# 0kam/alproj

Hardware: AMD Instinct MI355X
Metric: Gpoints/s projected (pinhole + Brown-Conrady, single pose) over the 100M-vertex DSM; CMA-ES iterations/s in `cma` (higher is better)
Workload: dtype f32

## Files before the change

### alproj_amd/_build.py

```python
import os
import shutil
import subprocess
import sys

HERE = os.path.dirname(os.path.abspath(__file__))
ROOT = os.path.dirname(HERE)
CSRC = os.path.join(HERE, "csrc")
INCLUDE = os.path.join(ROOT, "include")
BUILD = os.path.join(ROOT, "build")
LIB = os.path.join(HERE, "libalproj_hip.so")
SOURCES = ["alp_core.hip", "alp_points.hip", "alp_raster.hip", "alp_mesh.hip", "alp_rasterize.hip", "alp_sampler.hip",
           "alp_cma.hip", "alp_lm.hip", "host/alp_host.cpp"]
HOST_DIR = os.path.join(CSRC, "host")
HOST_SAN = os.path.join(BUILD, "host_san")
HOST_KINDS = {"plain": [], "asan": ["-fsanitize=address,undefined", "-fno-sanitize-recover=all"], "tsan": ["-fsanitize=thread"]}
EXTRA_FLAGS = {"alp_raster.hip": ["-ffp-contract=off"], "alp_mesh.hip": ["-ffp-contract=off"], "alp_cma.hip": ["-ffp-contract=off"],
               "alp_lm.hip": ["-ffp-contract=off"]}
ARCH = "gfx950"


def hipcc():
    exe = shutil.which("hipcc") or "/opt/rocm/bin/hipcc"
    if not os.path.exists(exe):
        raise RuntimeError("hipcc not found; libalproj_hip.so cannot be built")
    return exe


def _stale(target, deps):
    if not os.path.exists(target):
        return True
    t = os.path.getmtime(target)
    return any(os.path.getmtime(d) > t for d in deps)


# ... 38 lines not shown
        return shutil.which("g++")
    exe = "/opt/rocm/lib/llvm/bin/clang++"
    return exe if os.path.exists(exe) else shutil.which("amdclang++")


def build_host(kind="plain", compiler="clang", force=False):
    cxx = host_compiler(compiler)
    if not cxx:
        raise RuntimeError(f"no {compiler} C++ compiler found")
    os.makedirs(HOST_SAN, exist_ok=True)
    srcs = [os.path.join(HOST_DIR, f) for f in ("alp_host.cpp", "alp_host_selfcheck.cpp")]
    deps = srcs + [os.path.join(HOST_DIR, f) for f in ("alp_host.h", "alp_fold.h", "alp_plan.h", "alp_jacplan.h", "alp_lm.h", "alp_buffer.h")] + [os.path.join(INCLUDE, "alproj_hip.h"), os.path.abspath(__file__)]
    exe = os.path.join(HOST_SAN, f"alp_host_{kind}_{compiler}")
    if force or _stale(exe, deps):
        cmd = [cxx, "-O1", "-g", "-fno-omit-frame-pointer", "-std=c++17", "-ffp-contract=off", "-Wall", "-Wextra", f"-I{INCLUDE}", f"-I{CSRC}"] + \
              HOST_KINDS[kind] + srcs + ["-o", exe, "-lpthread"]
        r = subprocess.run(cmd, capture_output=True, text=True)
        if r.returncode != 0:
            sys.stderr.write(r.stderr)
            raise RuntimeError(f"{cxx} failed on the host-only build ({kind})")
    return exe


def resource_usage():
    out = {}
    for src in SOURCES:
        log = os.path.join(BUILD, os.path.basename(src).replace(".hip", ".o.log").replace(".cpp", ".o.log"))
        if not os.path.exists(log):
            continue
        cur = None
        for line in open(log):
            if "remark:" not in line or "[-Rpass-analysis" not in line:
                continue
            body = line.split("remark:", 1)[1].split("[-Rpass")[0].strip()
            if body.startswith("Function Name:"):
                cur = body.split(":", 1)[1].strip()
                out[cur] = {}
            elif cur and ":" in body:
                k, v = body.split(":", 1)
                out[cur][k.strip()] = v.strip()
    return out


if __name__ == "__main__":
    print(build(force="--force" in sys.argv, verbose=True))
    for k, v in resource_usage().items():
# ... 3 lines not shown
```

### alproj_amd/_lib.py

```python
import ctypes
import os
import threading
import weakref

import numpy as np

_HERE = os.path.dirname(os.path.abspath(__file__))
LIB_PATH = os.environ.get("ALPROJ_HIP_LIB", os.path.join(_HERE, "libalproj_hip.so"))

ALP_F32, ALP_F64, ALP_I32, ALP_I64, ALP_U8, ALP_U16 = 0, 1, 2, 3, 4, 5
LOSS_MEAN_DIST, LOSS_HUBER = 0, 1
NORMAL_LOSSES = {"linear": 0, "soft_l1": 1, "huber": 2, "cauchy": 3}
NORMAL_BATCH_MAX = 1024
WEIGHT_TABLE_MAX_BYTES = 1 << 30
NPARAM = 25
UNIQUE_ID_BYTES = 128

PARAM_KEYS = ("x", "y", "z", "fov", "pan", "tilt", "roll", "a1", "a2",
              "k1", "k2", "k3", "k4", "k5", "k6", "p1", "p2",
              "s1", "s2", "s3", "s4", "w", "h", "cx", "cy")
DIST_KEYS = PARAM_KEYS[7:21]


_POOL_MIN = 8 << 20
# ... 128 lines not shown
    "alp_synchronize": [],
    "alp_event_record": [_c_int],
    "alp_event_elapsed_ms": [_c_int, _c_int, _c_fp],
    "alp_kernel_timing": [_c_int],
    "alp_kernel_time_ms": [_c_fp, ctypes.POINTER(_c_int)],
    "alp_build_flags": [],
    "alp_comm_unique_id": [ctypes.c_char_p],
    "alp_comm_init": [ctypes.c_char_p, _c_int, _c_int],
    "alp_comm_destroy": [],
    "alp_comm_info": [ctypes.POINTER(_c_int), ctypes.POINTER(_c_int)],
    "alp_comm_bcast": [_c_void_p, _c_i64, _c_int],
    "alp_comm_allgather_counts": [_c_i64, ctypes.POINTER(_c_i64)],
    "alp_comm_allgatherv": [_c_void_p, _c_void_p, ctypes.POINTER(_c_i64)],
    "alp_points_create": [_c_void_p, _c_int, _c_i64, _c_dp, _c_int, ctypes.POINTER(_c_void_p)],
    "alp_points_create_columns": [_c_void_p, _c_void_p, _c_void_p, _c_int, _c_i64, _c_dp, _c_int, ctypes.POINTER(_c_void_p)],
    "alp_points_destroy": [_c_void_p],
    "alp_points_count": [_c_void_p, ctypes.POINTER(_c_i64)],
    "alp_points_layout": [_c_void_p, ctypes.POINTER(_c_i64)],
    "alp_points_set_observed": [_c_void_p, _c_void_p, _c_int],
    "alp_points_set_observed_columns": [_c_void_p, _c_void_p, _c_void_p, _c_int],
    "alp_project": [_c_void_p, _c_dp],
    "alp_projected_fetch": [_c_void_p, _c_void_p, _c_void_p, _c_int],
    "alp_projected_fetch_strided": [_c_void_p, _c_i64, _c_i64, _c_i64, _c_dp, _c_dp],
    "alp_residuals": [_c_void_p, _c_dp, _c_dp],
    "alp_residuals_batch": [_c_void_p, _c_dp, _c_i64, _c_dp],
    "alp_jacobian": [_c_void_p, _c_dp, ctypes.POINTER(ctypes.c_int32), _c_int, _c_int, _c_dp],
    "alp_normal_equations": [_c_void_p, _c_dp, ctypes.POINTER(ctypes.c_int32), _c_int, _c_int, _c_double, _c_dp],
    "alp_normal_equations_batch": [_c_void_p, _c_dp, _c_i64, ctypes.POINTER(ctypes.c_int32), _c_int, _c_int, _c_double, _c_dp],
    "alp_eval_population": [_c_void_p, _c_dp, _c_i64, _c_int, _c_double, _c_dp, ctypes.POINTER(_c_i64)],
    "alp_eval_population_enqueue": [_c_void_p, _c_dp, _c_i64, _c_int, _c_double],
    "alp_eval_population_wait": [_c_void_p, _c_dp, ctypes.POINTER(_c_i64)],
    "alp_eval_population_timing": [_c_void_p, _c_fp, _c_fp],
    "alp_eval_population_info": [_c_void_p, ctypes.POINTER(_c_i64)],
    "alp_points_set_mend": [_c_void_p, _c_int],
    "alp_points_set_weights": [_c_void_p, _c_void_p, _c_int],
    "alp_points_weight_sum": [_c_void_p, ctypes.POINTER(ctypes.c_double)],
    "alp_points_set_weight_table": [_c_void_p, _c_void_p, _c_int, _c_int],
    "alp_points_weight_table_sums": [_c_void_p, _c_dp],
    "alp_normal_equations_batch_rows": [_c_void_p, _c_dp, _c_i64, ctypes.POINTER(ctypes.c_int32), ctypes.POINTER(ctypes.c_int32), _c_int,
                                        _c_int, _c_double, _c_dp],
    "alp_residuals_assigned": [_c_void_p, _c_dp, _c_i64, ctypes.POINTER(ctypes.c_int32), _c_dp],
    "alp_eval_population_mended": [_c_void_p, ctypes.POINTER(_c_i64)],
    "alp_loss_uv": [_c_dp, _c_dp, _c_i64, _c_int, _c_double, _c_dp],
    "alp_loss_uv_columns": [_c_dp, _c_dp, _c_dp, _c_dp, _c_i64, _c_int, _c_double, _c_dp],
    "alp_cma_sample": [_c_dp, _c_double, _c_dp, _c_dp, _c_dp, _c_int, _c_i64, _c_int, ctypes.c_uint64, ctypes.c_uint64, _c_dp,
                       ctypes.POINTER(ctypes.c_int32)],
# ... 198 lines not shown
    return idx


def weights_check(w, n, precision=None):
    w = np.asarray(w)
    if w.dtype not in (np.float32, np.float64):
        w = w.astype(np.float64)
    w = np.ascontiguousarray(w)
    if w.shape != (n,):
        raise ValueError(f"weights must have shape ({n},)")
    if not np.isfinite(w).all() or (w < 0).any():
        raise ValueError("weights must be finite and >= 0")
    with np.errstate(over="ignore"):
        stored = w.astype(np.float32) if precision == ALP_F32 else w
    if not np.isfinite(stored).all():
        raise ValueError("a weight does not fit float32")
    world = _c_int()
    check(load().alp_comm_info(None, ctypes.byref(world)))
    if world.value == 1 and n > 0 and not stored.astype(np.float64).sum() > 0:
        raise ValueError("the weights sum to 0: no point is left")
    return w


class Points:

    def __init__(self, xyz, origin, precision="f32", _columns=None):
        l = lib()
        cols = _columns
        if cols is None:
            xyz = np.asarray(xyz)
            if xyz.ndim != 2 or xyz.shape[1] != 3:
                raise ValueError("xyz must have shape (N, 3)")
            if xyz.dtype not in (np.float32, np.float64):
                xyz = xyz.astype(np.float64)
            if not xyz.flags["C_CONTIGUOUS"] and xyz.shape[0] > 1 and all(xyz[:, k].flags["C_CONTIGUOUS"] for k in range(3)):
                cols = [xyz[:, k] for k in range(3)]
        self.precision = PRECISIONS[precision]
        self.origin = np.ascontiguousarray(origin, dtype=np.float64).reshape(3)
        h = _c_void_p()
        if cols is not None:
            cols = _same_float_columns(cols, 3)
            self.n = int(len(cols[0]))
            check(l.alp_points_create_columns(*[c.ctypes.data_as(_c_void_p) for c in cols], dtype_code(cols[0]), self.n,
                                              as_dp(self.origin), self.precision, ctypes.byref(h)))
        else:
            xyz = np.ascontiguousarray(xyz)
# ... 789 lines not shown
```

### alproj_amd/csrc/alp_core.hip

```cpp
#include "alp_internal.h"

#include <rccl/rccl.h>
#include <cmath>
#include <cstdlib>
#include <vector>

namespace alp {

Context &ctx() {
    static Context c;
    return c;
}

int require_init() {
    if (!ctx().ready) return fail(ALP_ENOTINIT, "alp_init has not been called (or failed)");
    return ALP_OK;
}

int scratch_reserve(size_t bytes, void **out) {
    Context &c = ctx();
    if (bytes > c.scratch_cap) {
        if (c.scratch) {
            ALP_HIP(hipStreamSynchronize(c.stream));
            hipFree(c.scratch);
// ... 75 lines not shown
    hipError_t e = hipGetDeviceCount(&n);
    if (e != hipSuccess || n <= 0)
        return fail(ALP_ENODEVICE, "no HIP device available (%s); libalproj_hip has no CPU fallback",
                    e == hipSuccess ? "device count is 0" : hipGetErrorString(e));
    if (device < 0 || device >= n)
        return fail(ALP_ENODEVICE, "device %d out of range (have %d)", device, n);
    ALP_HIP(hipSetDevice(device));
    hipDeviceProp_t prop;
    ALP_HIP(hipGetDeviceProperties(&prop, device));
    c.cu_count = prop.multiProcessorCount;
    ALP_HIP(hipStreamCreateWithFlags(&c.stream, hipStreamNonBlocking));
    for (auto &ev : c.events) ALP_HIP(hipEventCreate(&ev));
    c.device = device;
    c.ready = true;
    return ALP_OK;
}

int alp_shutdown(void) {
    Context &c = ctx();
    if (!c.ready) return ALP_OK;
    alp_comm_destroy();
    hipStreamSynchronize(c.stream);
    points_release_staging();
    if (c.scratch) hipFree(c.scratch);
    c.scratch = nullptr;
    c.scratch_cap = 0;
    for (auto &ev : c.events) {
        if (ev) hipEventDestroy(ev);
        ev = nullptr;
    }
    for (int i = 0; i < KT_MAX; ++i) {
        if (g_kt.a[i]) hipEventDestroy(g_kt.a[i]);
        if (g_kt.b[i]) hipEventDestroy(g_kt.b[i]);
        g_kt.a[i] = g_kt.b[i] = nullptr;
    }
    g_kt = KTimer();
    hipStreamDestroy(c.stream);
    c.stream = nullptr;
    c.ready = false;
    c.device = -1;
    return ALP_OK;
}

int alp_device_info(char *name, int len, int *cu_count, int64_t *hbm_bytes) {
    if (int rc = require_init()) return rc;
    hipDeviceProp_t prop;
// ... 194 lines not shown
```

### alproj_amd/csrc/alp_internal.h

```cpp
#pragma once

#include <hip/hip_runtime.h>

#include "host/alp_host.h"
#include "host/alp_buffer.h"

namespace alp {

#define ALP_HIP(expr)                                                                     \
    do {                                                                                  \
        hipError_t e__ = (expr);                                                          \
        if (e__ != hipSuccess)                                                            \
            return ::alp::fail(ALP_EHIP, "%s failed: %s (%s:%d)", #expr,                  \
                               hipGetErrorString(e__), __FILE__, __LINE__);               \
    } while (0)

struct DeviceMemory {
    static int alloc(void **p, size_t bytes) {
        const hipError_t e = hipMalloc(p, bytes);
        return e == hipSuccess ? ALP_OK : fail(ALP_EHIP, "hipMalloc of %zu bytes failed: %s", bytes, hipGetErrorString(e));
    }
    static void release(void *p) { hipFree(p); }
};
struct PinnedMemory {
// ... 31 lines not shown
    hipStream_t stream = nullptr;
    hipEvent_t events[64] = {};
    void *scratch = nullptr;
    size_t scratch_cap = 0;
    void *comm = nullptr;
    int rank = 0;
    int world = 1;
};
Context &ctx();
int require_init();
int scratch_reserve(size_t bytes, void **out);

void ktime_begin();
void ktime_end();
struct KTimeScope {
    KTimeScope() { ktime_begin(); }
    ~KTimeScope() { ktime_end(); }
};


const char *raster_dev_flags();

void points_release_staging();

int comm_allreduce_sum_f64(double *dev_buf, int64_t count);

}
```

### alproj_amd/csrc/alp_point_kernels.h

```cpp
#pragma once

#include "alp_internal.h"

namespace alp {

template <typename T> struct Num;
template <> struct Num<float> {
    using vec = float4;
    static constexpr int VEC = 4;
    static __device__ __forceinline__ float rcp(float a) { return __builtin_amdgcn_rcpf(a); }
    static __device__ __forceinline__ float sqrt(float a) { return __builtin_amdgcn_sqrtf(a); }
    static __device__ __forceinline__ float fma(float a, float b, float c) { return __builtin_fmaf(a, b, c); }
    static __device__ __forceinline__ float rcp_pop(float a) { return rcp(a); }
    static __device__ __forceinline__ float sqrt_pop(float a) { return sqrt(a); }
    typedef float native4 __attribute__((ext_vector_type(4)));
    static __device__ __forceinline__ float4 nt_load(const float4 *p) {
        const native4 t = __builtin_nontemporal_load(reinterpret_cast<const native4 *>(p));
        return make_float4(t.x, t.y, t.z, t.w);
    }
    static __device__ __forceinline__ float4 load(const float4 *p) {
        const native4 t = *reinterpret_cast<const native4 *>(p);
        return make_float4(t.x, t.y, t.z, t.w);
    }
    static __device__ __forceinline__ void nt_store(const float4 &a, float4 *p) {
// ... 643 lines not shown
                                                     const TS *__restrict__ uo, const TS *__restrict__ vo, int64_t n,
                                                     int64_t groups_per, double inv_f_scale, const JacPlan *__restrict__ plan,
                                                     double *__restrict__ partials, const TS *__restrict__ wts) {
    normal_body<TS, LOSS, WEIGHTED>(x, y, z, uo, vo, n, groups_per, inv_f_scale, plan, (int64_t)blockIdx.x, partials, (int64_t)blockIdx.x, wts);
}

constexpr int NORMAL_BATCH_POSE_IN_X = 1;
template <typename TS, int LOSS, bool WEIGHTED = false>
__global__ __launch_bounds__(256) void normal_poses_kernel(const TS *__restrict__ x, const TS *__restrict__ y, const TS *__restrict__ z,
                                                           const TS *__restrict__ uo, const TS *__restrict__ vo, int64_t n,
                                                           int64_t groups_per, double inv_f_scale, const JacPlan *__restrict__ plans,
                                                           const int *__restrict__ list, const long long *__restrict__ count,
                                                           int pose_in_x, double *__restrict__ partials, const TS *__restrict__ wts,
                                                           int64_t row_stride, const int *__restrict__ row_of_pose) {
    const int slot = pose_in_x ? blockIdx.x : blockIdx.y, stripe = pose_in_x ? blockIdx.y : blockIdx.x;
    const int stripes = pose_in_x ? gridDim.y : gridDim.x;
    if (count && (long long)slot >= *count) return;
    const int pose = list ? list[slot] : slot;
    if constexpr (WEIGHTED) wts += (int64_t)(row_of_pose ? row_of_pose[pose] : pose) * row_stride;
    normal_body<TS, LOSS, WEIGHTED>(x, y, z, uo, vo, n, groups_per, inv_f_scale, plans + pose, (int64_t)stripe, partials,
                                    (int64_t)pose * stripes + stripe, wts);
}

__global__ __launch_bounds__(256) void reduce_normal_poses_kernel(const double *__restrict__ partials, int stripes, int T, double n_local,
                                                                  const double *__restrict__ row_sums, const int *__restrict__ row_of_pose,
                                                                  const int *__restrict__ running, double *__restrict__ sums) {
    __shared__ double s[8][32];
    const int cl = threadIdx.x & 31;
    const int g = threadIdx.x >> 5;
    const int c = blockIdx.x * 32 + cl;
    const double *rows = partials + (int64_t)blockIdx.y * stripes * T;
    double *out = sums + (int64_t)blockIdx.y * (T + 1);
    const bool live = running ? running[blockIdx.y] != 0 : true;
    double acc = 0.0;
    if (c < T && live)
        for (int b = g; b < stripes; b += 8) acc += rows[(int64_t)b * T + c];
    s[g][cl] = acc;
    __syncthreads();
    if (g == 0 && c < T) {
        double t = s[0][cl];
#pragma unroll
        for (int k = 1; k < 8; ++k) t += s[k][cl];
        out[c] = t;
    }
    if (blockIdx.x == 0 && threadIdx.x == 0) out[T] = row_sums ? row_sums[row_of_pose ? row_of_pose[blockIdx.y] : (int)blockIdx.y] : n_local;
}


constexpr int64_t WT_SUM_CHUNK = 16384;
template <typename TIn>
__global__ __launch_bounds__(256) void weight_table_sums_kernel(const TIn *__restrict__ src, int64_t row_stride, int64_t len, int64_t chunk,
                                                                double *__restrict__ out) {
    __shared__ double s[256];
    const int tid = threadIdx.x;
    const int64_t beg = (int64_t)blockIdx.x * chunk;
    const int64_t end = beg + chunk < len ? beg + chunk : len;
    const TIn *row = src + (int64_t)blockIdx.y * row_stride;
    double acc = 0.0;
    for (int64_t i = beg + tid; i < end; i += 256) acc += (double)row[i];
    s[tid] = acc;
    __syncthreads();
    for (int m = 128; m >= 1; m >>= 1) {
        if (tid < m) s[tid] += s[tid + m];
        __syncthreads();
    }
    if (tid == 0) out[(int64_t)blockIdx.y * gridDim.x + blockIdx.x] = s[0];
}

constexpr int RA_LDS_POSES = 128;
// ... 147 lines not shown
template <typename T, int LOSS, typename Cfg = PopCfg<T>, bool SHARED_POSE = false, typename TS = T, bool LENS_FREE = false, bool WEIGHTED = false>
__global__ __launch_bounds__(256, Cfg::MINW) void popeval_kernel(
    const TS *__restrict__ x, const TS *__restrict__ y, const TS *__restrict__ z, const TS *__restrict__ uo,
    const TS *__restrict__ vo, int64_t n, const PoseRec<T> *__restrict__ cands, int P, T f_scale,
    double *__restrict__ partials, const PoseRec<T> *__restrict__ cands_general, const TS *__restrict__ wts) {
    popeval_body<T, LOSS, Cfg, SHARED_POSE, TS, LENS_FREE, WEIGHTED>(x, y, z, uo, vo, n, cands, P, f_scale, partials, cands_general, wts);
}

struct MendCount {
    long long last;
    long long total;
};

template <int LOSS, bool WEIGHTED = false>
__global__ __launch_bounds__(256, PopCfg<double>::MINW) void popeval_counted_kernel(
    const float *__restrict__ x, const float *__restrict__ y, const float *__restrict__ z, const float *__restrict__ uo,
    const float *__restrict__ vo, int64_t n, const PoseRec<double> *__restrict__ cands, const MendCount *__restrict__ cnt,
    double f_scale, double *__restrict__ partials, const float *__restrict__ wts) {
    const int count = (int)cnt->last;
    if ((int)blockIdx.y * PopCfg<double>::TC >= count) return;
    popeval_body<double, LOSS, PopCfg<double>, false, float, false, WEIGHTED>(x, y, z, uo, vo, n, cands, count, f_scale, partials, cands, wts);
}

__global__ __launch_bounds__(256) void mend_select_kernel(const double *__restrict__ sums, int P, const double *__restrict__ params,
                                                          double o0, double o1, double o2, int *__restrict__ idx,
                                                          PoseRec<double> *__restrict__ recs, MendCount *__restrict__ cnt) {
    __shared__ int s_wave[4];
    __shared__ int s_base;
    const int tid = threadIdx.x, lane = tid & 63, wave = tid >> 6;
    if (tid == 0) s_base = 0;
    __syncthreads();
    for (int c0 = 0; c0 < P; c0 += 256) {
        const int c = c0 + tid;
        const bool bad = c < P && (__builtin_bit_cast(unsigned long long, sums[c < P ? c : 0]) & 0x7ff0000000000000ull) == 0x7ff0000000000000ull;
        const unsigned long long m = __builtin_amdgcn_ballot_w64(bad);
        if (lane == 0) s_wave[wave] = __builtin_popcountll(m);
        __syncthreads();
        int before = s_base;
        for (int w = 0; w < wave; ++w) before += s_wave[w];
        if (bad) idx[before + __builtin_popcountll(m & ((1ull << lane) - 1ull))] = c;
        __syncthreads();
        if (tid == 0) s_base += (s_wave[0] + s_wave[1]) + (s_wave[2] + s_wave[3]);
        __syncthreads();
    }
    const int count = s_base;
    if (tid == 0) {
// ... 36 lines not shown
    if (k < (int)cnt->last) sums[idx[k]] = mended[k];
}

__global__ __launch_bounds__(256) void reduce_partials_kernel(const double *__restrict__ partials,
                                                              int nblk, int P, double n_local,
                                                              double *__restrict__ sums) {
    __shared__ double s[8][32];
    const int cl = threadIdx.x & 31;
    const int g = threadIdx.x >> 5;
    const int c = blockIdx.x * 32 + cl;
    double acc = 0.0;
    if (c < P)
        for (int b = g; b < nblk; b += 8) acc += partials[(int64_t)b * P + c];
    s[g][cl] = acc;
    __syncthreads();
    if (g == 0 && c < P) {
        double t = s[0][cl];
#pragma unroll
        for (int k = 1; k < 8; ++k) t += s[k][cl];
        sums[c] = t;
    }
    if (blockIdx.x == 0 && threadIdx.x == 0) sums[P] = n_local;
}

template <int LOSS, bool OBS_COLUMNS, bool PRJ_COLUMNS>
__global__ __launch_bounds__(256) void loss_uv_kernel(const double *__restrict__ obs_a, const double *__restrict__ obs_b,
                                                      const double *__restrict__ prj_a, const double *__restrict__ prj_b, int64_t n,
                                                      double f_scale, double *__restrict__ partials) {
    __shared__ double s[4];
    double acc = 0.0;
    const int64_t stride = (int64_t)gridDim.x * blockDim.x;
    for (int64_t i = (int64_t)blockIdx.x * blockDim.x + threadIdx.x; i < n; i += stride) {
        double2 o, q;
        if constexpr (OBS_COLUMNS) o = make_double2(obs_a[i], obs_b[i]);
        else o = reinterpret_cast<const double2 *>(obs_a)[i];
        if constexpr (PRJ_COLUMNS) q = make_double2(prj_a[i], prj_b[i]);
        else q = reinterpret_cast<const double2 *>(prj_a)[i];
        const double du = o.x - q.x, dv = o.y - q.y;
        const double r = __builtin_sqrt(du * du + dv * dv);
        if constexpr (LOSS == ALP_LOSS_MEAN_DIST) acc += r;
        else acc += (r <= f_scale) ? 0.5 * (r * r) : f_scale * (r - 0.5 * f_scale);
    }
    acc = wave_sum_to_lane63(acc);
    if ((threadIdx.x & 63) == 63) s[threadIdx.x >> 6] = acc;
    __syncthreads();
    if (threadIdx.x == 0) partials[blockIdx.x] = ((s[0] + s[1]) + s[2]) + s[3];
}

template <typename TIn, typename T, int C>
__global__ __launch_bounds__(256) void aos_to_planes_kernel(const TIn *__restrict__ src, int64_t count,
                                                            int64_t dst_off, double o0, double o1, double o2,
                                                            T *__restrict__ p0, T *__restrict__ p1,
                                                            T *__restrict__ p2) {
    const int64_t stride = (int64_t)gridDim.x * blockDim.x;
    for (int64_t i = (int64_t)blockIdx.x * blockDim.x + threadIdx.x; i < count; i += stride) {
        p0[dst_off + i] = (T)((double)src[i * C + 0] - o0);
        p1[dst_off + i] = (T)((double)src[i * C + 1] - o1);
        if constexpr (C == 3) p2[dst_off + i] = (T)((double)src[i * C + 2] - o2);
    }
}

template <typename T>
__global__ __launch_bounds__(256) void gather_strided_kernel(const T *__restrict__ u, const T *__restrict__ v,
                                                             int64_t first, int64_t stride, int64_t count,
                                                             double *__restrict__ out) {
    const int64_t i = (int64_t)blockIdx.x * blockDim.x + threadIdx.x;
    if (i < count) {
        out[i] = (double)u[first + i * stride];
        out[count + i] = (double)v[first + i * stride];
    }
}

}
```

### alproj_amd/optimize.py

```python
from contextlib import nullcontext
from math import cos, pi, sin, tan

import numpy as np
import pandas as pd
from scipy.optimize import least_squares
from tqdm import tqdm

from . import _lib, resample
from .cma import CMA

__all__ = ["intrinsic_mat", "extrinsic_mat", "project", "rmse", "huber_loss",
           "compute_residuals", "DEFAULT_BOUND_WIDTHS", "bounds_to_array", "BaseOptimizer",
           "CMAOptimizer", "LsqOptimizer", "start_seeds", "best_start", "normal_lm", "normal_lm_batch"]


def intrinsic_mat(fov_x_deg, w, h, cx=None, cy=None):
    if cx is None:
        cx = w / 2
    if cy is None:
        cy = h / 2
    half_x = fov_x_deg * pi / 180 / 2
    half_y = (fov_x_deg * pi / 180) * h / w / 2
    return np.array([[w / (2 * tan(half_x)), 0, cx],
                     [0, h / (2 * tan(half_y)), cy],
# ... 62 lines not shown
    if isinstance(uv, list):
        pts.set_observed_columns(uv[0], uv[1])
    else:
        pts.set_observed(uv)


def _as_rows(a):
    return np.ascontiguousarray(np.column_stack(a) if isinstance(a, list) else a, dtype=np.float64)


F64_MAX_POINTS = 4_000_000


def default_precision(n_points, precision=None):
    if precision is not None:
        if precision not in ("f32", "f64"):
            raise ValueError("precision must be None, 'f32' or 'f64'")
        return precision
    return "f64" if int(n_points) <= F64_MAX_POINTS else "f32"


def project(obj_points, params, precision="f64"):
    xyz = _xyz_array(obj_points)
    with _points(xyz, _camera_origin(params), precision) as pts:
        pts.project(_lib.params_vector(params))
        u, v = pts.fetch(np.float64)
    return pd.DataFrame({"u": u, "v": v}, copy=False)


def _uv_pointers(a):
    if isinstance(a, list):
        cols = [np.ascontiguousarray(c, dtype=np.float64) for c in a]
        return _lib.as_dp(cols[0]), _lib.as_dp(cols[1]), len(cols[0]), cols
    a = np.asarray(a, dtype=np.float64)
    if a.ndim != 2 or a.shape[1] != 2:
        raise ValueError("pixel coordinates must have shape (N, 2)")
    if not a.flags["C_CONTIGUOUS"] and a.shape[0] > 1 and a[:, 0].flags["C_CONTIGUOUS"] and a[:, 1].flags["C_CONTIGUOUS"]:
        cols = [a[:, 0], a[:, 1]]
        return _lib.as_dp(cols[0]), _lib.as_dp(cols[1]), a.shape[0], cols
    a = np.ascontiguousarray(a)
    return _lib.as_dp(a), None, a.shape[0], a


def _loss_uv(img_points, projected, kind, f_scale):
    prj = _first_two_columns(projected) if isinstance(projected, pd.DataFrame) else projected
    ou, ov, n_obs, keep_o = _uv_pointers(_uv_array(img_points))
    pu, pv, n_prj, keep_p = _uv_pointers(prj)
    if n_obs != n_prj:
        raise ValueError("img_points and projected must have the same shape")
# ... 702 lines not shown
```

### include/alproj_hip.h

```cpp
#ifndef ALPROJ_HIP_H
#define ALPROJ_HIP_H

#include <stdint.h>

#ifdef __cplusplus
extern "C" {
#endif

#define ALP_ABI_VERSION 7

#define ALP_NPARAM 25
#define ALP_PARAM_ORDER "x,y,z,fov,pan,tilt,roll,a1,a2,k1,k2,k3,k4,k5,k6,p1,p2,s1,s2,s3,s4,w,h,cx,cy"

enum alp_error {
    ALP_OK = 0,
    ALP_EINVAL = -1,
    ALP_ENOTINIT = -2,
    ALP_ENODEVICE = -3,
    ALP_EHIP = -4,
    ALP_ERCCL = -5,
    ALP_ESTATE = -6
};

enum alp_dtype {
// ... 44 lines not shown
int alp_comm_init(const char id[ALP_UNIQUE_ID_BYTES], int rank, int world_size);
int alp_comm_destroy(void);
int alp_comm_info(int *rank, int *world_size);
int alp_comm_bcast(void *buf, int64_t bytes, int root);
int alp_comm_allgather_counts(int64_t bytes, int64_t *counts);
int alp_comm_allgatherv(const void *send, void *recv, const int64_t *counts);

typedef struct alp_points alp_points_t;

int alp_points_create(const void *xyz, int in_dtype, int64_t n, const double origin[3],
                      int precision, alp_points_t **out);
int alp_points_create_columns(const void *x, const void *y, const void *z, int in_dtype, int64_t n,
                              const double origin[3], int precision, alp_points_t **out);
int alp_points_destroy(alp_points_t *pts);
int alp_points_count(const alp_points_t *pts, int64_t *n);
int alp_points_layout(const alp_points_t *pts, int64_t *row_length);
int alp_points_set_observed(alp_points_t *pts, const void *uv, int in_dtype);
int alp_points_set_observed_columns(alp_points_t *pts, const void *u, const void *v, int in_dtype);

int alp_project(alp_points_t *pts, const double params[ALP_NPARAM]);
int alp_projected_fetch(alp_points_t *pts, void *u_out, void *v_out, int out_dtype);
int alp_projected_fetch_strided(alp_points_t *pts, int64_t first, int64_t stride,
                                int64_t count, double *u_out, double *v_out);

int alp_residuals(alp_points_t *pts, const double params[ALP_NPARAM], double *out);
int alp_residuals_batch(alp_points_t *pts, const double *cand, int64_t B, double *out);
int alp_jacobian(alp_points_t *pts, const double params[ALP_NPARAM], const int32_t *target_idx, int D, int of_residuals,
                 double *out);
int alp_normal_equations(alp_points_t *pts, const double params[ALP_NPARAM], const int32_t *target_idx, int D, int loss,
                         double f_scale, double *out);
int alp_normal_equations_batch(alp_points_t *pts, const double *params, int64_t B, const int32_t *target_idx, int D, int loss,
                               double f_scale, double *out);
int alp_normal_equations_batch_rows(alp_points_t *pts, const double *params, int64_t B, const int32_t *row_of_pose,
                                    const int32_t *target_idx, int D, int loss, double f_scale, double *out);
int alp_residuals_assigned(alp_points_t *pts, const double *cand, int64_t B, const int32_t *assign, double *out);

int alp_eval_population(alp_points_t *pts, const double *cand, int64_t P, int loss_kind,
                        double f_scale, double *loss_out, int64_t *argmin_out);
int alp_eval_population_enqueue(alp_points_t *pts, const double *cand, int64_t P,
                                int loss_kind, double f_scale);
int alp_eval_population_wait(alp_points_t *pts, double *loss_out, int64_t *argmin_out);
int alp_eval_population_timing(alp_points_t *pts, float *kernel_ms, float *allreduce_ms);
enum alp_pop_variant { ALP_POP_GENERAL = 0, ALP_POP_SHARED_POSE = 1, ALP_POP_LENS_FREE = 2 };
int alp_eval_population_info(alp_points_t *pts, int64_t info[3]);
int alp_points_set_mend(alp_points_t *pts, int enable);
int alp_eval_population_mended(alp_points_t *pts, int64_t info[4]);
// ... 127 lines not shown
```

Measured before the change: 498.5.

## Stream one-shot projection through a chunked upload/kernel/download pipeline

Adds alp_project_table, which projects host points without building a persistent Points object. It splits the input into chunks over a three-slot device ring, with separate upload, kernel and download streams driven by host threads, so host-device copies overlap with projection. The kernel uses nontemporal loads and stores, and optional host conversion happens in pinned staging buffers. The aim is to remove the serial create, project and fetch path for single-pose projection, at the cost of extra threading and event complexity.

```diff
diff --git a/alproj_amd/_build.py b/alproj_amd/_build.py
--- a/alproj_amd/_build.py
+++ b/alproj_amd/_build.py
@@ -9,7 +9,7 @@
 INCLUDE = os.path.join(ROOT, "include")
 BUILD = os.path.join(ROOT, "build")
 LIB = os.path.join(HERE, "libalproj_hip.so")
-SOURCES = ["alp_core.hip", "alp_points.hip", "alp_raster.hip", "alp_mesh.hip", "alp_rasterize.hip", "alp_sampler.hip",
+SOURCES = ["alp_core.hip", "alp_points.hip", "alp_table.hip", "alp_raster.hip", "alp_mesh.hip", "alp_rasterize.hip", "alp_sampler.hip",
            "alp_cma.hip", "alp_lm.hip", "host/alp_host.cpp"]
 HOST_DIR = os.path.join(CSRC, "host")
 HOST_SAN = os.path.join(BUILD, "host_san")
@@ -94,6 +94,22 @@
     return exe
 
 
+def build_table_plan(kind="plain", compiler="clang", force=False):
+    cxx = host_compiler(compiler)
+    if not cxx:
+        raise RuntimeError(f"no {compiler} C++ compiler found")
+    os.makedirs(HOST_SAN, exist_ok=True)
+    src = os.path.join(HOST_DIR, "alp_table_selfcheck.cpp")
+    exe = os.path.join(HOST_SAN, f"alp_table_plan_{kind}_{compiler}")
+    if force or _stale(exe, [src, os.path.join(HOST_DIR, "alp_table_plan.h"), os.path.abspath(__file__)]):
+        cmd = [cxx, "-O1", "-g", "-fno-omit-frame-pointer", "-std=c++17", "-Wall", "-Wextra", f"-I{CSRC}"] + HOST_KINDS[kind] + [src, "-o", exe]
+        r = subprocess.run(cmd, capture_output=True, text=True)
+        if r.returncode != 0:
+            sys.stderr.write(r.stderr)
+            raise RuntimeError(f"{cxx} failed on the table-plan driver ({kind})")
+    return exe
+
+
 def resource_usage():
     out = {}
     for src in SOURCES:
diff --git a/alproj_amd/_lib.py b/alproj_amd/_lib.py
--- a/alproj_amd/_lib.py
+++ b/alproj_amd/_lib.py
@@ -174,6 +174,7 @@
     "alp_project": [_c_void_p, _c_dp],
     "alp_projected_fetch": [_c_void_p, _c_void_p, _c_void_p, _c_int],
     "alp_projected_fetch_strided": [_c_void_p, _c_i64, _c_i64, _c_i64, _c_dp, _c_dp],
+    "alp_project_table": [_c_void_p, _c_void_p, _c_void_p, _c_void_p, _c_int, _c_i64, _c_dp, _c_dp, _c_int, _c_void_p, _c_void_p, _c_int, _c_i64],
     "alp_residuals": [_c_void_p, _c_dp, _c_dp],
     "alp_residuals_batch": [_c_void_p, _c_dp, _c_i64, _c_dp],
     "alp_jacobian": [_c_void_p, _c_dp, ctypes.POINTER(ctypes.c_int32), _c_int, _c_int, _c_dp],
@@ -418,6 +419,36 @@
     return w
 
 
+def project_table(xyz, origin, pvec, precision="f64", dtype=np.float64, chunk_points=0):
+    l = lib()
+    cols = None
+    if isinstance(xyz, (list, tuple)):
+        cols = xyz
+    else:
+        xyz = np.asarray(xyz)
+        if xyz.ndim != 2 or xyz.shape[1] != 3:
+            raise ValueError("xyz must have shape (N, 3)")
+        if xyz.dtype not in (np.float32, np.float64):
+            xyz = xyz.astype(np.float64)
+        if not xyz.flags["C_CONTIGUOUS"] and xyz.shape[0] > 1 and all(xyz[:, k].flags["C_CONTIGUOUS"] for k in range(3)):
+            cols = [xyz[:, k] for k in range(3)]
+    origin = np.ascontiguousarray(origin, dtype=np.float64).reshape(3)
+    pvec = np.ascontiguousarray(pvec, dtype=np.float64)
+    if cols is not None:
+        cols = _same_float_columns(cols, 3)
+        n, code = int(len(cols[0])), dtype_code(cols[0])
+        src = [None] + [c.ctypes.data_as(_c_void_p) for c in cols]
+    else:
+        xyz = np.ascontiguousarray(xyz)
+        n, code = int(xyz.shape[0]), dtype_code(xyz)
+        src = [xyz.ctypes.data_as(_c_void_p), None, None, None]
+    u = result_empty(n, dtype)
+    v = result_empty(n, dtype)
+    check(l.alp_project_table(*src, code, n, as_dp(origin), as_dp(pvec), PRECISIONS[precision], u.ctypes.data_as(_c_void_p),
+                              v.ctypes.data_as(_c_void_p), dtype_code(u), int(chunk_points)))
+    return u, v
+
+
 class Points:
 
     def __init__(self, xyz, origin, precision="f32", _columns=None):
diff --git a/alproj_amd/csrc/alp_core.hip b/alproj_amd/csrc/alp_core.hip
--- a/alproj_amd/csrc/alp_core.hip
+++ b/alproj_amd/csrc/alp_core.hip
@@ -121,6 +121,7 @@
     alp_comm_destroy();
     hipStreamSynchronize(c.stream);
     points_release_staging();
+    table_release();
     if (c.scratch) hipFree(c.scratch);
     c.scratch = nullptr;
     c.scratch_cap = 0;
diff --git a/alproj_amd/csrc/alp_internal.h b/alproj_amd/csrc/alp_internal.h
--- a/alproj_amd/csrc/alp_internal.h
+++ b/alproj_amd/csrc/alp_internal.h
@@ -77,6 +77,7 @@
 const char *raster_dev_flags();
 
 void points_release_staging();
+void table_release();
 
 int comm_allreduce_sum_f64(double *dev_buf, int64_t count);
 
diff --git a/alproj_amd/csrc/alp_point_kernels.h b/alproj_amd/csrc/alp_point_kernels.h
--- a/alproj_amd/csrc/alp_point_kernels.h
+++ b/alproj_amd/csrc/alp_point_kernels.h
@@ -689,6 +689,7 @@
                                     (int64_t)pose * stripes + stripe, wts);
 }
 
+#ifndef ALP_POINT_KERNELS_TEMPLATES_ONLY
 __global__ __launch_bounds__(256) void reduce_normal_poses_kernel(const double *__restrict__ partials, int stripes, int T, double n_local,
                                                                   const double *__restrict__ row_sums, const int *__restrict__ row_of_pose,
                                                                   const int *__restrict__ running, double *__restrict__ sums) {
@@ -712,6 +713,7 @@
     }
     if (blockIdx.x == 0 && threadIdx.x == 0) out[T] = row_sums ? row_sums[row_of_pose ? row_of_pose[blockIdx.y] : (int)blockIdx.y] : n_local;
 }
+#endif
 
 
 constexpr int64_t WT_SUM_CHUNK = 16384;
@@ -905,6 +907,7 @@
     popeval_body<double, LOSS, PopCfg<double>, false, float, false, WEIGHTED>(x, y, z, uo, vo, n, cands, count, f_scale, partials, cands, wts);
 }
 
+#ifndef ALP_POINT_KERNELS_TEMPLATES_ONLY
 __global__ __launch_bounds__(256) void mend_select_kernel(const double *__restrict__ sums, int P, const double *__restrict__ params,
                                                           double o0, double o1, double o2, int *__restrict__ idx,
                                                           PoseRec<double> *__restrict__ recs, MendCount *__restrict__ cnt) {
@@ -987,6 +990,7 @@
     }
     if (blockIdx.x == 0 && threadIdx.x == 0) sums[P] = n_local;
 }
+#endif
 
 template <int LOSS, bool OBS_COLUMNS, bool PRJ_COLUMNS>
 __global__ __launch_bounds__(256) void loss_uv_kernel(const double *__restrict__ obs_a, const double *__restrict__ obs_b,
@@ -1025,6 +1029,60 @@
     }
 }
 
+typedef uint32_t raw16 __attribute__((ext_vector_type(4)));
+typedef uint32_t raw8 __attribute__((ext_vector_type(2)));
+
+template <typename E, int COUNT>
+__device__ __forceinline__ void nt_load_run(const E *p, E (&out)[COUNT]) {
+    constexpr int BYTES = COUNT * (int)sizeof(E);
+    static_assert(BYTES % 8 == 0, "a lane's share is whole 8-byte words");
+    if constexpr (BYTES % 16 == 0) {
+        raw16 raw[BYTES / 16];
+#pragma unroll
+        for (int j = 0; j < BYTES / 16; ++j) raw[j] = __builtin_nontemporal_load(reinterpret_cast<const raw16 *>(p) + j);
+        __builtin_memcpy(out, raw, BYTES);
+    } else {
+        raw8 raw[BYTES / 8];
+#pragma unroll
+        for (int j = 0; j < BYTES / 8; ++j) raw[j] = __builtin_nontemporal_load(reinterpret_cast<const raw8 *>(p) + j);
+        __builtin_memcpy(out, raw, BYTES);
+    }
+}
+
+template <typename TIn, typename T, bool ROWS>
+__global__ __launch_bounds__(256) void project_table_kernel(const TIn *__restrict__ src, int64_t plane, T *__restrict__ u,
+                                                            T *__restrict__ v, int64_t nvec, double o0, double o1, double o2,
+                                                            PoseRec<T> pose) {
+    using Vt = typename Num<T>::vec;
+    constexpr int NP = Num<T>::VEC;
+    const int64_t i = (int64_t)blockIdx.x * blockDim.x + threadIdx.x;
+    if (i >= nvec) return;
+    TIn c[3][NP];
+    if constexpr (ROWS) {
+        TIn run[3 * NP];
+        nt_load_run<TIn, 3 * NP>(src + i * (3 * NP), run);
+#pragma unroll
+        for (int k = 0; k < NP; ++k) {
+            c[0][k] = run[3 * k];
+            c[1][k] = run[3 * k + 1];
+            c[2][k] = run[3 * k + 2];
+        }
+    } else {
+#pragma unroll
+        for (int a = 0; a < 3; ++a) nt_load_run<TIn, NP>(src + a * plane + i * NP, c[a]);
+    }
+    Vt ou, ov;
+#pragma unroll
+    for (int k = 0; k < NP; ++k) {
+        const T qx = (T)((double)c[0][k] - o0), qy = (T)((double)c[1][k] - o1), qz = (T)((double)c[2][k] - o2);
+        T xd, yd;
+        project_norm<T>(pose.v, qx, qy, qz, xd, yd);
+        to_pixels<T>(pose.v, xd, yd, vget<T>(ou, k), vget<T>(ov, k));
+    }
+    Num<T>::nt_store(ou, reinterpret_cast<Vt *>(u) + i);
+    Num<T>::nt_store(ov, reinterpret_cast<Vt *>(v) + i);
+}
+
 template <typename T>
 __global__ __launch_bounds__(256) void gather_strided_kernel(const T *__restrict__ u, const T *__restrict__ v,
                                                              int64_t first, int64_t stride, int64_t count,
diff --git a/alproj_amd/csrc/alp_table.hip b/alproj_amd/csrc/alp_table.hip
--- /dev/null
+++ b/alproj_amd/csrc/alp_table.hip
@@ -0,0 +1,277 @@
+#include "alp_internal.h"
+
+#include <condition_variable>
+#include <mutex>
+#include <thread>
+
+#define ALP_POINT_KERNELS_TEMPLATES_ONLY
+#include "alp_point_kernels.h"
+#include "host/alp_table_plan.h"
+
+using namespace alp;
+
+namespace {
+
+constexpr int S = host::TABLE_SLOTS;
+constexpr size_t IN_BYTES = 24, OUT_BYTES = 16;
+
+struct TableRings {
+    hipStream_t up = nullptr, down = nullptr;
+    hipEvent_t ev_up[S] = {}, ev_kern[S] = {}, ev_down[S] = {};
+    char *in = nullptr, *out = nullptr;
+    int64_t slot_points = 0;
+    char *stage[2] = {nullptr, nullptr};
+    int64_t stage_points = 0;
+} g_tab;
+
+int ensure_streams() {
+    TableRings &g = g_tab;
+    if (!g.up) ALP_HIP(hipStreamCreateWithFlags(&g.up, hipStreamNonBlocking));
+    if (!g.down) ALP_HIP(hipStreamCreateWithFlags(&g.down, hipStreamNonBlocking));
+    for (hipEvent_t *evs : {g.ev_up, g.ev_kern, g.ev_down})
+        for (int s = 0; s < S; ++s)
+            if (!evs[s]) ALP_HIP(hipEventCreateWithFlags(&evs[s], hipEventDisableTiming));
+    return ALP_OK;
+}
+
+int sync_streams() {
+    hipError_t e = hipStreamSynchronize(ctx().stream), e2 = g_tab.up ? hipStreamSynchronize(g_tab.up) : hipSuccess,
+               e3 = g_tab.down ? hipStreamSynchronize(g_tab.down) : hipSuccess;
+    e = e != hipSuccess ? e : (e2 != hipSuccess ? e2 : e3);
+    return e == hipSuccess ? ALP_OK : fail(ALP_EHIP, "alp_project_table: %s", hipGetErrorString(e));
+}
+
+int ensure_rings(int64_t points) {
+    TableRings &g = g_tab;
+    if (points <= g.slot_points) return ALP_OK;
+    if (int rc = sync_streams()) return rc;
+    g.slot_points = 0;
+    if (g.in) hipFree(g.in);
+    if (g.out) hipFree(g.out);
+    g.in = g.out = nullptr;
+    ALP_HIP(hipMalloc((void **)&g.in, (size_t)points * IN_BYTES * S));
+    ALP_HIP(hipMalloc((void **)&g.out, (size_t)points * OUT_BYTES * S));
+    ALP_HIP(hipMemsetAsync(g.in, 0, (size_t)points * IN_BYTES * S, ctx().stream));
+    ALP_HIP(hipMemsetAsync(g.out, 0, (size_t)points * OUT_BYTES * S, ctx().stream));
+    ALP_HIP(hipStreamSynchronize(ctx().stream));
+    g.slot_points = points;
+    return ALP_OK;
+}
+
+int ensure_stage(int64_t points) {
+    TableRings &g = g_tab;
+    if (points <= g.stage_points) return ALP_OK;
+    g.stage_points = 0;
+    for (auto &b : g.stage) {
+        if (b) hipHostFree(b);
+        b = nullptr;
+        ALP_HIP(hipHostMalloc((void **)&b, (size_t)points * OUT_BYTES, hipHostMallocDefault));
+    }
+    g.stage_points = points;
+    return ALP_OK;
+}
+
+struct Pipe {
+    std::mutex m;
+    std::condition_variable cv;
+    int64_t up = 0, kern = 0, down = 0;
+    hipError_t err = hipSuccess;
+    const char *where = nullptr;
+
+    bool wait(const int64_t &counter, int64_t above) {
+        std::unique_lock<std::mutex> l(m);
+        cv.wait(l, [&] { return counter > above || err != hipSuccess; });
+        return err == hipSuccess;
+    }
+    void advance(int64_t &counter) {
+        {
+            std::lock_guard<std::mutex> l(m);
+            ++counter;
+        }
+        cv.notify_all();
+    }
+    void failed(hipError_t e, const char *what) {
+        {
+            std::lock_guard<std::mutex> l(m);
+            if (err == hipSuccess) err = e, where = what;
+        }
+        cv.notify_all();
+    }
+};
+
+#define TAB_HIP(expr, what)                \
+    do {                                   \
+        hipError_t e__ = (expr);           \
+        if (e__ != hipSuccess) {           \
+            p.failed(e__, what);           \
+            return;                        \
+        }                                  \
+    } while (0)
+
+struct TableCall {
+    const char *rows = nullptr;
+    const char *cols[3] = {};
+    size_t in_es = 0, t_es = 0, out_es = 0;
+    int64_t n = 0, chunk = 0, jobs = 0;
+    double origin[3] = {}, rec[POSE_WORDS] = {};
+    char *out[2] = {};
+    void (*launch)(const TableCall &, const void *src, void *u, void *v, int64_t cnt) = nullptr;
+    void (*convert)(const void *src, void *dst, int64_t n, int threads) = nullptr;
+    int threads = 1;
+};
+
+template <typename TIn, typename T, bool ROWS>
+void launch_chunk(const TableCall &c, const void *src, void *u, void *v, int64_t cnt) {
+    PoseRec<T> pose;
+    for (int i = 0; i < POSE_WORDS; ++i) pose.v[i] = (T)c.rec[i];
+    const int64_t nvec = (cnt + Num<T>::VEC - 1) / Num<T>::VEC;
+    hipLaunchKernelGGL((project_table_kernel<TIn, T, ROWS>), dim3((unsigned)((nvec + 255) / 256)), dim3(256), 0, ctx().stream,
+                       (const TIn *)src, g_tab.slot_points, (T *)u, (T *)v, nvec, c.origin[0], c.origin[1], c.origin[2], pose);
+}
+
+template <typename S_, typename D>
+void convert_chunk(const void *src, void *dst, int64_t n, int threads) {
+    host::convert_threads((const S_ *)src, (D *)dst, n, threads);
+}
+
+char *in_slot(int slot) { return g_tab.in + (size_t)slot * g_tab.slot_points * IN_BYTES; }
+char *out_slot(int slot) { return g_tab.out + (size_t)slot * g_tab.slot_points * OUT_BYTES; }
+char *out_slot_v(const TableCall &c, int slot) { return out_slot(slot) + (size_t)g_tab.slot_points * c.t_es; }
+
+void stage_up(Pipe &p, const TableCall &c) {
+    TableRings &g = g_tab;
+    TAB_HIP(hipSetDevice(ctx().device), "hipSetDevice");
+    for (int64_t k = 0; k < c.jobs; ++k) {
+        const host::TableJob j = host::table_job(k, c.n, c.chunk);
+        if (!p.wait(p.kern, k - S)) return;
+        if (k >= S) TAB_HIP(hipStreamWaitEvent(g.up, g.ev_kern[j.slot], 0), "copy up: wait for the slot's kernel");
+        char *dst = in_slot(j.slot);
+        if (c.rows)
+            TAB_HIP(hipMemcpyAsync(dst, c.rows + (size_t)j.off * 3 * c.in_es, (size_t)j.cnt * 3 * c.in_es, hipMemcpyHostToDevice, g.up), "copy up");
+        else
+            for (int a = 0; a < 3; ++a)
+                TAB_HIP(hipMemcpyAsync(dst + (size_t)a * g.slot_points * c.in_es, c.cols[a] + (size_t)j.off * c.in_es, (size_t)j.cnt * c.in_es,
+                                       hipMemcpyHostToDevice, g.up), "copy up");
+        TAB_HIP(hipEventRecord(g.ev_up[j.slot], g.up), "copy up: event");
+        p.advance(p.up);
+    }
+}
+
+void stage_kernel(Pipe &p, const TableCall &c) {
+    TableRings &g = g_tab;
+    hipStream_t st = ctx().stream;
+    for (int64_t k = 0; k < c.jobs; ++k) {
+        const host::TableJob j = host::table_job(k, c.n, c.chunk);
+        if (!p.wait(p.up, k)) return;
+        TAB_HIP(hipStreamWaitEvent(st, g.ev_up[j.slot], 0), "kernel: wait for the copy up");
+        if (!p.wait(p.down, k - S)) return;
+        if (k >= S) TAB_HIP(hipStreamWaitEvent(st, g.ev_down[j.slot], 0), "kernel: wait for the slot's copy down");
+        c.launch(c, in_slot(j.slot), out_slot(j.slot), out_slot_v(c, j.slot), j.cnt);
+        TAB_HIP(hipGetLastError(), "project_table_kernel");
+        TAB_HIP(hipEventRecord(g.ev_kern[j.slot], st), "kernel: event");
+        p.advance(p.kern);
+    }
+}
+
+void stage_down(Pipe &p, const TableCall &c) {
+    TableRings &g = g_tab;
+    TAB_HIP(hipSetDevice(ctx().device), "hipSetDevice");
+    for (int64_t k = 0; k <= c.jobs; ++k) {
+        if (k < c.jobs) {
+            const host::TableJob j = host::table_job(k, c.n, c.chunk);
+            if (!p.wait(p.kern, k)) return;
+            TAB_HIP(hipStreamWaitEvent(g.down, g.ev_kern[j.slot], 0), "copy down: wait for the kernel");
+            const size_t bytes = (size_t)j.cnt * c.t_es;
+            char *du = c.convert ? g.stage[k & 1] : c.out[0] + (size_t)j.off * c.out_es;
+            char *dv = c.convert ? g.stage[k & 1] + bytes : c.out[1] + (size_t)j.off * c.out_es;
+            TAB_HIP(hipMemcpyAsync(du, out_slot(j.slot), bytes, hipMemcpyDeviceToHost, g.down), "copy down");
+            TAB_HIP(hipMemcpyAsync(dv, out_slot_v(c, j.slot), bytes, hipMemcpyDeviceToHost, g.down), "copy down");
+            TAB_HIP(hipEventRecord(g.ev_down[j.slot], g.down), "copy down: event");
+            p.advance(p.down);
+        }
+        if (c.convert && k > 0) {
+            const host::TableJob j = host::table_job(k - 1, c.n, c.chunk);
+            TAB_HIP(hipEventSynchronize(g.ev_down[j.slot]), "copy down: wait for the chunk");
+            const char *src = g.stage[(k - 1) & 1];
+            c.convert(src, c.out[0] + (size_t)j.off * c.out_es, j.cnt, c.threads);
+            c.convert(src + (size_t)j.cnt * c.t_es, c.out[1] + (size_t)j.off * c.out_es, j.cnt, c.threads);
+        }
+    }
+}
+
+int run_pipeline(const TableCall &c) {
+    Pipe p;
+    std::thread up(stage_up, std::ref(p), std::cref(c)), down(stage_down, std::ref(p), std::cref(c));
+    stage_kernel(p, c);
+    up.join();
+    down.join();
+    const int rc = sync_streams();
+    if (p.err != hipSuccess) return fail(ALP_EHIP, "alp_project_table: %s: %s", p.where, hipGetErrorString(p.err));
+    return rc;
+}
+
+}
+
+namespace alp {
+void table_release() {
+    TableRings &g = g_tab;
+    if (g.up) hipStreamSynchronize(g.up);
+    if (g.down) hipStreamSynchronize(g.down);
+    if (g.in) hipFree(g.in);
+    if (g.out) hipFree(g.out);
+    for (auto &b : g.stage)
+        if (b) hipHostFree(b);
+    for (hipEvent_t *evs : {g.ev_up, g.ev_kern, g.ev_down})
+        for (int s = 0; s < S; ++s)
+            if (evs[s]) hipEventDestroy(evs[s]);
+    if (g.up) hipStreamDestroy(g.up);
+    if (g.down) hipStreamDestroy(g.down);
+    g = TableRings();
+}
+}
+
+extern "C" {
+
+int alp_project_table(const void *xyz, const void *x, const void *y, const void *z, int in_dtype, int64_t n, const double origin[3],
+                      const double params[ALP_NPARAM], int precision, void *u_out, void *v_out, int out_dtype, int64_t chunk_points) {
+    if (int rc = require_init()) return rc;
+    ALP_REQUIRE(n >= 0, "n is negative");
+    ALP_REQUIRE(origin && params, "origin or params is NULL");
+    ALP_REQUIRE(precision == ALP_F32 || precision == ALP_F64, "precision must be ALP_F32 or ALP_F64");
+    ALP_REQUIRE(in_dtype == ALP_F32 || in_dtype == ALP_F64, "in_dtype must be ALP_F32 or ALP_F64");
+    ALP_REQUIRE(out_dtype == ALP_F32 || out_dtype == ALP_F64, "out_dtype must be ALP_F32 or ALP_F64");
+    ALP_REQUIRE(chunk_points >= 0, "chunk_points is negative");
+    if (n == 0) return ALP_OK;
+    ALP_REQUIRE(xyz || (x && y && z), "coordinates are NULL");
+    ALP_REQUIRE(u_out && v_out, "output is NULL");
+
+    TableCall c;
+    c.rows = (const char *)xyz;
+    if (!xyz) c.cols[0] = (const char *)x, c.cols[1] = (const char *)y, c.cols[2] = (const char *)z;
+    c.in_es = in_dtype == ALP_F64 ? 8 : 4;
+    c.t_es = precision == ALP_F64 ? 8 : 4;
+    c.out_es = out_dtype == ALP_F64 ? 8 : 4;
+    c.n = n;
+    c.chunk = host::table_chunk_points(chunk_points);
+    c.jobs = host::table_job_count(n, c.chunk);
+    memcpy(c.origin, origin, sizeof(c.origin));
+    fold_pose(params, origin, c.rec);
+    c.out[0] = (char *)u_out;
+    c.out[1] = (char *)v_out;
+    using Launch = void (*)(const TableCall &, const void *, void *, void *, int64_t);
+    static const Launch launches[2][2][2] = {
+        {{launch_chunk<float, float, false>, launch_chunk<float, float, true>}, {launch_chunk<float, double, false>, launch_chunk<float, double, true>}},
+        {{launch_chunk<double, float, false>, launch_chunk<double, float, true>}, {launch_chunk<double, double, false>, launch_chunk<double, double, true>}}};
+    c.launch = launches[in_dtype == ALP_F64][precision == ALP_F64][xyz != nullptr];
+    if (out_dtype != precision) c.convert = out_dtype == ALP_F64 ? convert_chunk<float, double> : convert_chunk<double, float>;
+    c.threads = std::min(host::fetch_threads(), 14);
+
+    if (int rc = ensure_streams()) return rc;
+    const int64_t slot_points = host::table_slot_points(n, c.chunk);
+    if (int rc = ensure_rings(slot_points)) return rc;
+    if (c.convert)
+        if (int rc = ensure_stage(slot_points)) return rc;
+    return run_pipeline(c);
+}
+
+}
diff --git a/alproj_amd/csrc/host/alp_table_plan.h b/alproj_amd/csrc/host/alp_table_plan.h
--- /dev/null
+++ b/alproj_amd/csrc/host/alp_table_plan.h
@@ -0,0 +1,40 @@
+#pragma once
+
+#include <cstdint>
+
+namespace alp {
+namespace host {
+
+constexpr int TABLE_SLOTS = 3;
+constexpr int64_t TABLE_CHUNK_UNIT = 1024;
+constexpr int64_t TABLE_CHUNK_MAX = (int64_t)8 << 20;
+constexpr int64_t TABLE_CHUNK_DEFAULT = (int64_t)1 << 20;
+
+inline int64_t table_chunk_points(int64_t request) {
+    if (request <= 0) return TABLE_CHUNK_DEFAULT;
+    if (request > TABLE_CHUNK_MAX) return TABLE_CHUNK_MAX;
+    return (request + TABLE_CHUNK_UNIT - 1) / TABLE_CHUNK_UNIT * TABLE_CHUNK_UNIT;
+}
+
+inline int64_t table_slot_points(int64_t n, int64_t chunk) {
+    const int64_t need = n < chunk ? (n < 1 ? 1 : n) : chunk;
+    return (need + TABLE_CHUNK_UNIT - 1) / TABLE_CHUNK_UNIT * TABLE_CHUNK_UNIT;
+}
+
+inline int64_t table_job_count(int64_t n, int64_t chunk) { return n <= 0 ? 0 : (n + chunk - 1) / chunk; }
+
+struct TableJob {
+    int64_t off, cnt;
+    int slot;
+};
+
+inline TableJob table_job(int64_t k, int64_t n, int64_t chunk) {
+    TableJob j;
+    j.off = k * chunk;
+    j.cnt = n - j.off < chunk ? n - j.off : chunk;
+    j.slot = (int)(k % TABLE_SLOTS);
+    return j;
+}
+
+}
+}
diff --git a/alproj_amd/csrc/host/alp_table_selfcheck.cpp b/alproj_amd/csrc/host/alp_table_selfcheck.cpp
--- /dev/null
+++ b/alproj_amd/csrc/host/alp_table_selfcheck.cpp
@@ -0,0 +1,77 @@
+#include <cstdio>
+#include <cstdlib>
+#include <cstring>
+#include <vector>
+
+#include "host/alp_table_plan.h"
+
+using namespace alp::host;
+
+namespace {
+
+int g_bad = 0;
+#define CHECK(cond, ...)                                  \
+    do {                                                  \
+        if (!(cond)) {                                    \
+            if (++g_bad <= 20) {                          \
+                fprintf(stderr, "CHECK FAILED %s: ", #cond); \
+                fprintf(stderr, __VA_ARGS__);             \
+                fprintf(stderr, "\n");                    \
+            }                                             \
+        }                                                 \
+    } while (0)
+
+void check_plan(int64_t n, int64_t request) {
+    const int64_t chunk = table_chunk_points(request);
+    CHECK(chunk >= TABLE_CHUNK_UNIT && chunk <= TABLE_CHUNK_MAX && chunk % TABLE_CHUNK_UNIT == 0, "request %lld -> chunk %lld", (long long)request, (long long)chunk);
+    CHECK(request <= 0 ? chunk == TABLE_CHUNK_DEFAULT : (request > TABLE_CHUNK_MAX || (chunk >= request && chunk - request < TABLE_CHUNK_UNIT)),
+          "request %lld -> chunk %lld", (long long)request, (long long)chunk);
+    const int64_t slot_points = table_slot_points(n, chunk), jobs = table_job_count(n, chunk);
+    CHECK(slot_points % TABLE_CHUNK_UNIT == 0 && slot_points >= TABLE_CHUNK_UNIT && slot_points <= chunk, "n %lld chunk %lld -> slot %lld", (long long)n, (long long)chunk, (long long)slot_points);
+    CHECK((n <= 0) == (jobs == 0), "n %lld -> %lld jobs", (long long)n, (long long)jobs);
+    std::vector<int64_t> in_slot(TABLE_SLOTS, -1);
+    int64_t next = 0;
+    for (int64_t k = 0; k < jobs; ++k) {
+        const TableJob j = table_job(k, n, chunk);
+        CHECK(j.off == next, "n %lld chunk %lld job %lld starts at %lld, not %lld", (long long)n, (long long)chunk, (long long)k, (long long)j.off, (long long)next);
+        CHECK(j.cnt >= 1 && j.cnt <= slot_points, "job %lld of n %lld chunk %lld holds %lld points, a slot %lld", (long long)k, (long long)n, (long long)chunk, (long long)j.cnt, (long long)slot_points);
+        CHECK(k == jobs - 1 || j.cnt % TABLE_CHUNK_UNIT == 0, "job %lld of %lld holds %lld points", (long long)k, (long long)jobs, (long long)j.cnt);
+        CHECK(j.slot >= 0 && j.slot < TABLE_SLOTS, "slot %d", j.slot);
+        if (j.slot >= 0 && j.slot < TABLE_SLOTS) {
+            CHECK(in_slot[(size_t)j.slot] == (k < TABLE_SLOTS ? -1 : k - TABLE_SLOTS), "job %lld meets chunk %lld in slot %d", (long long)k, (long long)in_slot[(size_t)j.slot], j.slot);
+            in_slot[(size_t)j.slot] = k;
+        }
+        next = j.off + j.cnt;
+    }
+    CHECK(next == (n > 0 ? n : 0), "n %lld chunk %lld: the jobs end at %lld", (long long)n, (long long)chunk, (long long)next);
+}
+
+}
+
+int main(int argc, char **argv) {
+    if (argc == 4 && !strcmp(argv[1], "--plan")) {
+        const int64_t n = atoll(argv[2]), chunk = table_chunk_points(atoll(argv[3])), jobs = table_job_count(n, chunk);
+        printf("chunk %lld slot_points %lld jobs %lld\n", (long long)chunk, (long long)table_slot_points(n, chunk), (long long)jobs);
+        for (int64_t k = 0; k < jobs; ++k) {
+            const TableJob j = table_job(k, n, chunk);
+            printf("%lld %lld %lld %d\n", (long long)k, (long long)j.off, (long long)j.cnt, j.slot);
+        }
+        return 0;
+    }
+    const int64_t requests[] = {-5, 0, 1, 1000, 1023, 1024, 1025, 2048, 3000, 65536, TABLE_CHUNK_DEFAULT - 1, TABLE_CHUNK_DEFAULT, TABLE_CHUNK_DEFAULT + 1,
+                                TABLE_CHUNK_MAX, TABLE_CHUNK_MAX + 1, (int64_t)1 << 40};
+    for (int64_t request : requests) {
+        const int64_t chunk = table_chunk_points(request);
+        std::vector<int64_t> ns = {-1, 0, 1, 2, 3, 255, 1023, 1024, 1025, 100000000};
+        for (int64_t m = 1; m <= 7; ++m)
+            for (int64_t d = -1; d <= 1; ++d) ns.push_back(m * chunk + d);
+        for (int64_t d : {-1025, -1024, -1023, 7, 1023, 1024, 1025}) ns.push_back(5 * chunk + d);
+        for (int64_t n : ns) check_plan(n, request);
+    }
+    if (g_bad) {
+        fprintf(stderr, "%d checks failed\n", g_bad);
+        return 1;
+    }
+    printf("table plan ok\n");
+    return 0;
+}
diff --git a/alproj_amd/optimize.py b/alproj_amd/optimize.py
--- a/alproj_amd/optimize.py
+++ b/alproj_amd/optimize.py
@@ -108,9 +108,7 @@
 
 def project(obj_points, params, precision="f64"):
     xyz = _xyz_array(obj_points)
-    with _points(xyz, _camera_origin(params), precision) as pts:
-        pts.project(_lib.params_vector(params))
-        u, v = pts.fetch(np.float64)
+    u, v = _lib.project_table(xyz, _camera_origin(params), _lib.params_vector(params), precision, np.float64)
     return pd.DataFrame({"u": u, "v": v}, copy=False)
 
 
diff --git a/include/alproj_hip.h b/include/alproj_hip.h
--- a/include/alproj_hip.h
+++ b/include/alproj_hip.h
@@ -90,6 +90,9 @@
 int alp_projected_fetch(alp_points_t *pts, void *u_out, void *v_out, int out_dtype);
 int alp_projected_fetch_strided(alp_points_t *pts, int64_t first, int64_t stride,
                                 int64_t count, double *u_out, double *v_out);
+int alp_project_table(const void *xyz, const void *x, const void *y, const void *z, int in_dtype, int64_t n,
+                      const double origin[3], const double params[ALP_NPARAM], int precision, void *u_out, void *v_out,
+                      int out_dtype, int64_t chunk_points);
 
 int alp_residuals(alp_points_t *pts, const double params[ALP_NPARAM], double *out);
 int alp_residuals_batch(alp_points_t *pts, const double *cand, int64_t B, double *out);
```

After: 496.5. About the same (-0.4%).
